# ilirlikalla/Smith-Waterman-FPGA-module

Hardware: AMD Instinct MI355X
Metric: GCUPS (higher is better)
Workload: dtype f16

## Files before the change

smith-waterman-fpga-module_amd/csrc/swbank_f16_rows.inc:

```
#define SWK_F16M_L_Z0_L0 \
  "v_perm_b32 %[S1], %[nv], %[tb0], %[sel]\n\t" \
  "v_pk_add_f16 %[Db], %[h0], %[S1] clamp\n\t" \
  "v_pk_add_f16 %[DN], %[Da], %[no]\n\t" \
  "v_pk_maximum3_f16 %[h0], %[Da], %[up], %[t0]\n\t" \
  "v_pk_maximum3_f16 %[X], %[DN], %[up], %[t0]\n\t" \
  "v_perm_b32 %[S1], %[nv], %[tb1], %[sel]\n\t" \
  "v_pk_add_f16 %[DN], %[Db], %[no]\n\t" \
  "v_pk_add_f16 %[t0], %[X], %[ne]\n\t" \
  "v_pk_add_f16 %[Da], %[h1], %[S1] clamp\n\t" \
  "v_pk_maximum3_f16 %[h1], %[Db], %[t0], %[t1]\n\t" \
  "v_pk_maximum3_f16 %[X], %[DN], %[t0], %[t1]\n\t" \
  "v_pk_maximum3_f16 %[best], %[best], %[h0], %[h1]\n\t" \
  "v_perm_b32 %[S1], %[nv], %[tb2], %[sel]\n\t" \
  "v_pk_add_f16 %[DN], %[Da], %[no]\n\t" \
  "v_pk_add_f16 %[t1], %[X], %[ne]\n\t" \
  "v_pk_add_f16 %[Db], %[h2], %[S1] clamp\n\t" \
  "v_pk_maximum3_f16 %[h2], %[Da], %[t1], %[t2]\n\t" \
  "v_pk_maximum3_f16 %[X], %[DN], %[t1], %[t2]\n\t" \
  "v_perm_b32 %[S1], %[nv], %[tb3], %[sel]\n\t" \
  "v_pk_add_f16 %[DN], %[Db], %[no]\n\t" \
  "v_pk_add_f16 %[t2], %[X], %[ne]\n\t" \
  "v_pk_add_f16 %[Da], %[h3], %[S1] clamp\n\t" \
  "v_pk_maximum3_f16 %[h3], %[Db], %[t2], %[t3]\n\t" \
  "v_pk_maximum3_f16 %[X], %[DN], %[t2], %[t3]\n\t" \
// ... 1417 lines not shown
  "v_pk_add_f16 %[Db], %[h2], %[p2]\n\t" \
  "v_pk_maximum3_f16 %[b0], %[b0], %[m1], %[h1]\n\t" \
  "v_pk_maximum3_f16 %[t2], %[AO], %[t1], %[t2]\n\t" \
  "v_pk_add_f16 %[AO], %[Db], %[no]\n\t" \
  "v_pk_maximum3_f16 %[h2], %[t2], %[Da], %[c2]\n\t" \
  "v_pk_add_f16 %[Da], %[h3], %[p3]\n\t" \
  "v_pk_maximum3_f16 %[b1], %[b1], %[m2], %[h2]\n\t" \
  "v_pk_maximum3_f16 %[t3], %[AO], %[t2], %[t3]\n\t" \
  "v_pk_add_f16 %[b1], %[b1], %[e1]\n\t" \
  "v_pk_add_f16 %[AO], %[Da], %[no]\n\t" \
  "v_pk_maximum3_f16 %[b1], %[b1], %[g3], %[k3]\n\t" \
  "v_pk_maximum3_f16 %[h3], %[t3], %[Db], %[c3]\n\t" \
  "v_pk_add_f16 %[Db], %[h4], %[p4]\n\t" \
  "v_pk_maximum3_f16 %[b1], %[b1], %[m3], %[h3]\n\t" \
  "v_pk_maximum3_f16 %[t4], %[AO], %[t3], %[t4]\n\t" \
  "v_pk_add_f16 %[AO], %[Db], %[no]\n\t" \
  "v_pk_maximum3_f16 %[h4], %[t4], %[Da], %[c4]\n\t" \
  "v_pk_add_f16 %[Da], %[h5], %[p5]\n\t" \
  "v_pk_maximum3_f16 %[b2], %[b2], %[m4], %[h4]\n\t" \
  "v_pk_maximum3_f16 %[t5], %[AO], %[t4], %[t5]\n\t" \
  "v_pk_add_f16 %[b2], %[b2], %[e1]\n\t" \
  "v_pk_add_f16 %[AO], %[Da], %[no]\n\t" \
  "v_pk_maximum3_f16 %[b2], %[b2], %[g5], %[k5]\n\t" \
  "v_pk_maximum3_f16 %[h5], %[t5], %[Db], %[c5]\n\t" \
  "v_pk_add_f16 %[Db], %[h6], %[p6]\n\t" \
  "v_pk_maximum3_f16 %[b2], %[b2], %[m5], %[h5]\n\t" \
  "v_pk_maximum3_f16 %[t6], %[AO], %[t5], %[t6]\n\t" \
  "v_pk_add_f16 %[AO], %[Db], %[no]\n\t" \
  "v_pk_maximum3_f16 %[h6], %[t6], %[Da], %[c6]\n\t" \
  "v_pk_maximum3_f16 %[t7], %[AO], %[t6], %[t7]\n\t" \
  "v_pk_maximum3_f16 %[b3], %[b3], %[m6], %[h6]\n\t" \
  "v_pk_maximum3_f16 %[h7], %[t7], %[Db], %[c7]\n\t" \
  ""
#define SWK_F16M_F_Z0_L0 \
  "v_pk_fma_f16 %[Db], %[fa0], %[fb0], %[h0] op_sel:[0,1,0] op_sel_hi:[1,0,1] clamp\n\t" \
  "v_pk_add_f16 %[DN], %[Da], %[no]\n\t" \
  "v_pk_maximum3_f16 %[h0], %[Da], %[up], %[t0]\n\t" \
  "v_pk_maximum3_f16 %[X], %[DN], %[up], %[t0]\n\t" \
  "v_pk_add_f16 %[DN], %[Db], %[no]\n\t" \
  "v_pk_add_f16 %[t0], %[X], %[ne]\n\t" \
  "v_pk_fma_f16 %[Da], %[fa1], %[fb1], %[h1] op_sel:[0,1,0] op_sel_hi:[1,0,1] clamp\n\t" \
  "v_pk_maximum3_f16 %[h1], %[Db], %[t0], %[t1]\n\t" \
  "v_pk_maximum3_f16 %[X], %[DN], %[t0], %[t1]\n\t" \
  "v_pk_maximum3_f16 %[best], %[best], %[h0], %[h1]\n\t" \
  "v_pk_add_f16 %[DN], %[Da], %[no]\n\t" \
  "v_pk_add_f16 %[t1], %[X], %[ne]\n\t" \
  "v_pk_fma_f16 %[Db], %[fa2], %[fb2], %[h2] op_sel:[0,1,0] op_sel_hi:[1,0,1] clamp\n\t" \
  "v_pk_maximum3_f16 %[h2], %[Da], %[t1], %[t2]\n\t" \
  "v_pk_maximum3_f16 %[X], %[DN], %[t1], %[t2]\n\t" \
  "v_pk_add_f16 %[DN], %[Db], %[no]\n\t" \
  "v_pk_add_f16 %[t2], %[X], %[ne]\n\t" \
  "v_pk_fma_f16 %[Da], %[fa3], %[fb3], %[h3] op_sel:[0,1,0] op_sel_hi:[1,0,1] clamp\n\t" \
  "v_pk_maximum3_f16 %[h3], %[Db], %[t2], %[t3]\n\t" \
  "v_pk_maximum3_f16 %[X], %[DN], %[t2], %[t3]\n\t" \
  "v_pk_maximum3_f16 %[best], %[best], %[h2], %[h3]\n\t" \
  "v_pk_add_f16 %[DN], %[Da], %[no]\n\t" \
  "v_pk_add_f16 %[t3], %[X], %[ne]\n\t" \
  "v_pk_fma_f16 %[Db], %[fa4], %[fb4], %[h4] op_sel:[0,1,0] op_sel_hi:[1,0,1] clamp\n\t" \
  "v_pk_maximum3_f16 %[h4], %[Da], %[t3], %[t4]\n\t" \
  "v_pk_maximum3_f16 %[X], %[DN], %[t3], %[t4]\n\t" \
  "v_pk_add_f16 %[DN], %[Db], %[no]\n\t" \
  "v_pk_add_f16 %[t4], %[X], %[ne]\n\t" \
  "v_pk_fma_f16 %[Da], %[fa5], %[fb5], %[h5] op_sel:[0,1,0] op_sel_hi:[1,0,1] clamp\n\t" \
  "v_pk_maximum3_f16 %[h5], %[Db], %[t4], %[t5]\n\t" \
  "v_pk_maximum3_f16 %[X], %[DN], %[t4], %[t5]\n\t" \
  "v_pk_maximum3_f16 %[best], %[best], %[h4], %[h5]\n\t" \
// ... 372 lines not shown
```

smith-waterman-fpga-module_amd/csrc/swbank_internal.h:

```cpp
#ifndef SWBANK_INTERNAL_H
#define SWBANK_INTERNAL_H

#define SWB_MAX_QUERY 65536u
#define SWB_TILE 128
#define SWB_SEL_PAD 0x0Du
#define SWB_SEL_ZERO 0x0Cu

#define SWB_RECORD 64
#define SWB_RECORD_MAX 232u

#define SWK_PACK_BYTES 0u
#define SWK_PACK_RECORDS 1u
#define SWK_PACK_STREAM 2u
#define SWK_PACK_NIBBLE 3u
#define SWK_PACK_MIXED 4u

typedef struct SwkWaveSplit {
  unsigned pairs, P;
  const unsigned* qtab;
  const unsigned* fb_qtab;
  unsigned words, fb_words, PS, fb_PS;
  void* ring;
  unsigned cols;
  unsigned* prog;
  unsigned* fault;
  unsigned poll_limit, stall;
  unsigned wbal_blocks, wbal_grid, wbal_gen;
  unsigned wbal_waves;
  unsigned* wbal_flag;
  unsigned* wbal_state;
} SwkWaveSplit;

static inline int swk_wbal_admissible(unsigned long long U, unsigned long long B, unsigned W,
                                      unsigned grid) {
  return (W == 4 || W == 8) && grid != 0 && U * B >= 4ull * W * grid;
}

#define SWK_SKEW_ACC 4
#define SWK_BAL_WORDS(R, ACC) (2 * (R) + 1 + (ACC))

#define SWK_FAULT_BAL 1u
#define SWK_FAULT_TAIL 2u
#define SWK_FAULT_WBAL 4u
#define SWK_FAULT_WORDS 4


typedef struct SwkStreamChunk {
  unsigned tile0, res_off_lo, res_off_hi, zero_off256;
} SwkStreamChunk;
#define SWK_STREAM_ABORT 0xFFFFFFFFu

#define SWK_DEAL_MAX 16
typedef struct SwkDeal {
  unsigned D, stride;
  unsigned char* codes[SWK_DEAL_MAX];
  unsigned long long* offs[SWK_DEAL_MAX];
  unsigned* lens[SWK_DEAL_MAX];
  const int* scores[SWK_DEAL_MAX];
  unsigned long long cnt[SWK_DEAL_MAX];
  unsigned nib;
} SwkDeal;

#ifdef __cplusplus
extern "C"
#endif
int swbank_codon_table(const unsigned char* user, unsigned char out[64]);

#ifdef __cplusplus
extern "C" hipError_t swk_launch_stream(int R, int gotoh, int f16, int pair, const uint8_t* res,
                                        size_t n, uint32_t ulen, const SwkStreamChunk* sc,
                                        const uint32_t* hflag, uint32_t* dflag, uint32_t nsc,
// ... 15 lines not shown
```

smith-waterman-fpga-module_amd/csrc/swbank_ktile.hip:

```cpp
#include "swbank_kcommon.h"

namespace swk {

template <int C>
__device__ __forceinline__ void tile_chunks_local(const Lane2& t, size_t tlo, size_t thi, size_t n,
                                                  int lane, int& nch, int& nfull, int& ncl) {
  uint32_t Lmax = max(t.llo, t.lhi);
  uint32_t Lmin = min(tlo < n ? t.llo : ~0u, thi < n ? t.lhi : ~0u);
  uint32_t ol = (uint32_t)lane;
  asm volatile("" : "+v"(ol));
#pragma unroll
  for (int off = 32; off >= 1; off >>= 1) {
    const int ad = (int)((ol ^ (uint32_t)off) << 2);
    Lmax = max(Lmax, (uint32_t)__builtin_amdgcn_ds_bpermute(ad, (int)Lmax));
    Lmin = min(Lmin, (uint32_t)__builtin_amdgcn_ds_bpermute(ad, (int)Lmin));
  }
  const int lx = (int)__builtin_amdgcn_readfirstlane(Lmax);
  nch = max(1, (lx + C - 1) / C);
  ncl = lx == 0 ? C : lx - C * (nch - 1);
  const uint32_t lm = __builtin_amdgcn_readfirstlane(Lmin);
  nfull = lm == ~0u ? 0 : (int)(lm / C);
}

template <int R, int RB, bool COL0, bool PROF, bool GOTOH, bool F16, bool PAIR = false,
          bool MQ = false, bool STREAM = false, int C = 8, bool BAL = false, bool TRIM = false,
          bool SKEW = false>
__global__ void __launch_bounds__(R >= 64 ? 512 : 1024) score_kernel(const ScoreArgs a) {
  static_assert(!BAL || (!MQ && !STREAM && !COL0), "balanced ranges: one query, resident batch");
  static_assert(!TRIM || (BAL && PAIR), "trimmed last chunks: the balanced pair kernel");
  static_assert(!SKEW || (PAIR && F16 && !GOTOH && !MQ && !STREAM && R == 32 && C == 8),
                "SKEW: the merged f16 pair rows, one query, resident batch");
  static_assert(!MQ || !PROF, "several queries: row-LUT or pair-table variants");
  static_assert(!STREAM || (!MQ && !PROF), "streamed batches: single-query LUT / pair variants");
  static_assert(C == 8 || (C == 4 && PAIR && !STREAM), "4-column chunks: pair tables only");
  static_assert(!PAIR || ((R == 32 || (R == 16 && GOTOH)) && F16 && !PROF && !COL0 &&
                          (!GOTOH || !MQ)),
                "PAIR: f16, merged R = 32 or Gotoh R = 16 / 32 (one query)");
  extern __shared__ __attribute__((aligned(16))) uint32_t smem[];
  const int lane = threadIdx.x & 63;
  const int wave = __builtin_amdgcn_readfirstlane(threadIdx.x >> 6);
  const int W = __builtin_amdgcn_readfirstlane(blockDim.x >> 6);
  const bool seg_in = a.edge_in != nullptr, seg_out = a.edge_out != nullptr;
  uint32_t* bestsh = smem + (PAIR ? a.PS / 4 : 0);
  constexpr int RS = SWK_RING_ROW;
  uint2* ein = reinterpret_cast<uint2*>(bestsh + W * SWB_TILE);
  uint2* ring = ein + (seg_in ? 2 * C * RS : 0);
  uint8_t* prof = reinterpret_cast<uint8_t*>(ring + (size_t)(W > 1 ? 2 * (W - 1) : 1) * C * RS);

  size_t n = a.n;
  const uint32_t* idx = a.idx;
  if (idx && a.ident && __builtin_amdgcn_readfirstlane(*a.ident)) idx = nullptr;
  const uint32_t* sidx = TRIM ? a.sidx : nullptr;
  if (TRIM && sidx && a.ident && __builtin_amdgcn_readfirstlane(*a.ident)) sidx = nullptr;
  if (idx) {
    const uint32_t cnt = __builtin_amdgcn_readfirstlane(*a.nidx);
    n = cnt > a.idx_base ? min(a.n, (size_t)(cnt - a.idx_base)) : 0;
  }
  const int ntiles = (int)((n + SWB_TILE - 1) / SWB_TILE);
  const int G = (int)gridDim.x;
// ... 85 lines not shown
      return lane_targets<true>(base + (((size_t)scn * 12 + 15) & ~(size_t)15),
                                reinterpret_cast<const uint64_t*>(co), cl, scn, t - st0, lane, pk,
                                cperm, 0u, 0u);
    }
    return lane_targets<true>(base, nullptr, nullptr, scn, t - st0, lane, pk, nullptr, a.ulen,
                               pk == SWK_PACK_NIBBLE ? (a.ulen + 1) / 2 : (a.ulen + 3) / 4);
  };

  int unit = blockIdx.x, q = 0;
  int tile = unit;
  int vc0 = 0, vend = 0;
  if constexpr (BAL) {
    bal_visit(0, tile, vc0, vend);
    unit = tile;
  }
  if constexpr (MQ) {
    if (unit < nunits) {
      q = PAIR ? unit % (int)a.nq : unit / ntiles;
      tile = PAIR ? unit / (int)a.nq : unit - q * ntiles;
    }
  }
  Lane2 cur;
  if constexpr (STREAM) {
    cur = stream_tile(tile, packed);
    wperm = cperm;
    wst0 = st0;
  } else {
    cur = lane_targets<!MQ>(a.res, a.offs, a.lens, n, tile, lane, packed, idx, a.ulen,
                            a.ustride);
  }
  int nch, nfull, ncl;
  if constexpr (SKEW)
    tile_chunks_local<C>(cur, (size_t)tile * SWB_TILE + lane, (size_t)tile * SWB_TILE + lane + 64,
                         n, lane, nch, nfull, ncl);
  else
    tile_chunks<C>(cur, (size_t)tile * SWB_TILE + lane, (size_t)tile * SWB_TILE + lane + 64, n,
                   nch, nfull, ncl);
  (void)ncl;
  if constexpr (BAL) {
    if (vend >= 0 && vend < nch) ncl = C;
    nch = vend < 0 ? nch : vend;
  }
  const uint32_t S = a.S;

  for (int i = threadIdx.x; i < W * SWB_TILE; i += blockDim.x) bestsh[i] = 0;
  const f16x2 NOE2 = as_f16x2(as_u16x2(a.f16_noe)), NE2 = as_f16x2(as_u16x2(a.f16_ne)),
              NO2 = as_f16x2(as_u16x2(a.f16_no));
  typedef __attribute__((address_space(4))) const uint32_t cst_u32;
  cst_u32* const ct = reinterpret_cast<cst_u32*>(reinterpret_cast<uintptr_t>(a.ctab));
  constexpr uint32_t SKEW_NEG = 0xBC00BC00u;
  constexpr int NB = SKEW ? SWK_SKEW_ACC : 1;
  static_assert(NB == 1 || NB == 4, "the generated rows fold into 4 accumulators");
  uint32_t skew_c0 = 0;
  if constexpr (SKEW) skew_c0 = ct[1];
  const auto skew_reset = [&](u16x2 (&H)[R], u16x2 (&X)[R], u16x2 (&bk)[NB], u16x2& pup) {
    uint32_t c0 = skew_c0;
    asm volatile("" : "+v"(c0));
    f16x2 h = as_f16x2(__builtin_bit_cast(u16x2, c0));
    const f16x2 ne = as_f16x2(as_u16x2(a.f16_ne));
#pragma unroll
    for (int r = 0; r < R; ++r) {
      if (r < 8) {
        H[r] = as_u16x2(h);
        h = h - ne;
      } else {
        H[r] = H[r - 8];
      }
      X[r] = __builtin_bit_cast(u16x2, SKEW_NEG);
    }
    pup = H[7];
    if constexpr (NB == 4) {
      bk[0] = H[1];
      bk[1] = H[3];
      bk[2] = H[5];
      bk[3] = H[6];
    }
  };
  (void)ct; (void)skew_reset;
  if (wave == 0) {
    if (lane < C)
      ring[lane * RS + 64] = F16 ? make_uint2(0u, GOTOH ? 0u : as_u32(as_u16x2(NOE2)))
                                 : make_uint2(S | (S << 16), 0u);
    if (seg_in)
      dma_edge_chunk<C>(a.edge_in + (size_t)(MQ ? unit : tile) * a.ecols * 64, ein, lane);
  }
  uint32_t nv = a.nv;
  uint32_t tab[PROF || PAIR ? 1 : R];
  if constexpr (PAIR) {
    const uint4* src = reinterpret_cast<const uint4*>(a.qtab + (MQ ? (size_t)q * a.qwords : 0));
    for (uint32_t i = threadIdx.x; i < a.PS / 16; i += blockDim.x)
      reinterpret_cast<uint4*>(smem)[i] = src[i];
  } else if constexpr (PROF) {
    const uint32_t words = (a.pad + 1) * a.PS / 16;
    const uint4* src = reinterpret_cast<const uint4*>(a.qtab);
    for (uint32_t i = threadIdx.x; i < words; i += blockDim.x)
      reinterpret_cast<uint4*>(prof)[i] = src[i];
  } else {
    asm volatile("" : "+v"(nv));
#pragma unroll
    for (int r = 0; r < R; ++r)
      tab[r] = __builtin_amdgcn_readfirstlane(a.qtab[(MQ ? (size_t)q * a.qwords : 0) + wave * R + r]);
  }
  const u16x2 S2 = {(unsigned short)S, (unsigned short)S};
  const u16x2 O2 = {(unsigned short)a.O, (unsigned short)a.O};
  const u16x2 E2 = {(unsigned short)a.E, (unsigned short)a.E};
  const uint32_t oes = a.O + a.E + S;
  const u16x2 OES2 = {(unsigned short)oes, (unsigned short)oes};
  const u16x2 H0 = F16 ? (u16x2){0, 0} : S2;
  const u16x2 X0 = (F16 && !GOTOH) ? as_u16x2(NOE2) : (u16x2){0, 0};

  u16x2 Hl[R], Xl[R];
#pragma unroll
  for (int r = 0; r < R; ++r) {
    Hl[r] = H0;
    Xl[r] = X0;
// ... 140 lines not shown
            if (lane == 0) {
              sq[(k + 1) % W] = nt;
              if (nt >= ntiles) sq[W] = g + 1;
            }
            nunit = nt;
          } else {
            nunit = __builtin_amdgcn_readfirstlane(sq[(k + 1) % W]);
          }
        }
      }
      int ntile = nunit, nqq = q;
      if constexpr (MQ) {
        if (nunit < nunits) {
          if constexpr (PAIR) {
            ntile = nunit / (int)a.nq;
          } else {
            ntile = tile + G;
            while (ntile >= ntiles) {
              ntile -= ntiles;
              ++nqq;
            }
          }
        }
      }
      if (!last) {
        load_raw<C, !MQ>(cur, c + 1, c + 1 < nfull, a.pad, packed, rlo, rhi);
      } else if (nunit < nunits) {
        if constexpr (STREAM) cur = stream_tile(ntile, packed_n);
        else
          cur = lane_targets<!MQ>(a.res, a.offs, a.lens, n, ntile, lane, packed, idx, a.ulen,
                                  a.ustride);
        if constexpr (SKEW)
          tile_chunks_local<C>(cur, (size_t)ntile * SWB_TILE + lane,
                               (size_t)ntile * SWB_TILE + lane + 64, n, lane, nch_n, nfull_n, ncl_n);
        else
          tile_chunks<C>(cur, (size_t)ntile * SWB_TILE + lane,
                         (size_t)ntile * SWB_TILE + lane + 64, n, nch_n, nfull_n, ncl_n);
        if (BAL && nvend >= 0 && nvend < nch_n) ncl_n = C;
        if (BAL && nvend < 0) nvend = nch_n;
        load_raw<C, !MQ>(cur, nc0, nc0 < nfull_n, a.pad, STREAM ? packed_n : packed, rlo, rhi);
      }
      const int slot = g & 1;
      if (seg_in && wave == 0 && (last ? nunit < nunits : (MQ ? unit : tile) < nunits))
        dma_edge_chunk<C>(a.edge_in + ((size_t)(last ? nunit : MQ ? unit : tile) * a.ecols +
                                    (size_t)(last ? 0 : c + 1) * C) * 64,
                       ein + (size_t)((g + 1) & 1) * C * RS, lane);
      int rl = lane;
      if constexpr (SKEW) asm volatile("" : "+v"(rl));
      uint2* rin = wave > 0 ? ring + ((size_t)((wave - 1) * 2 + slot) * C) * RS + rl
                   : seg_in ? ein + (size_t)slot * C * RS + rl
                            : ring + 64;
      uint2* rout = wave < W - 1 ? ring + ((size_t)(wave * 2 + slot) * C) * RS + rl
                    : W > 1      ? rin
                                 : ring + rl;
      const int cu = __builtin_amdgcn_readfirstlane(c);
      uint32_t cs[SKEW ? 7 + C : 1];
      if constexpr (SKEW) {
        cst_u32* const sl = ct + (cu * C + 2);
#pragma unroll
        for (int s = 0; s < 7 + C; ++s) cs[s] = sl[s];
        if (wave == 0 && lane == 0) {
#pragma unroll
          for (int jj = 0; jj < C; ++jj) ring[jj * RS + 64] = make_uint2(cs[jj + 7], SKEW_NEG);
        }
      }
      (void)cu; (void)cs;
      uint2 rv = rin[0];
      ProfLookup16<PROF && F16 ? R : 2> lkq;
      (void)lkq;
      const int ncols = TRIM && c + 1 == nch ? ncl : C;
      bool trimmed = false;
      (void)ncols;
#pragma unroll
      for (int jj = 0; jj < C; ++jj) {
        if (TRIM && jj > 0 && __builtin_expect(jj >= ncols, 0)) {
          trimmed = true;
          break;
        }
        const u16x2 upH = as_u16x2(rv.x);
        u16x2 upX = as_u16x2(rv.y);
        if (jj + 1 < C) rv = rin[(jj + 1) * RS];
        u16x2 diag = prevUpH;
        prevUpH = upH;
        const uint32_t wlo = jj < 4 ? clo.x : clo.y, whi = jj < 4 ? chi.x : chi.y;
        if constexpr (PROF && F16) {
          const auto load16 = [&](int j, ProfLookup16<R>& out) {
            const uint32_t wl = j < 4 ? clo.x : clo.y, wh = j < 4 ? chi.x : chi.y;
            const uint32_t blo = min((wl >> (8 * (j & 3))) & 0xFFu, padc);
            const uint32_t bhi = min((wh >> (8 * (j & 3))) & 0xFFu, padc);
            const uint4* plo = reinterpret_cast<const uint4*>(prof + __umul24(blo, a.PS) + 2 * pbase);
            const uint4* phi = reinterpret_cast<const uint4*>(prof + __umul24(bhi, a.PS) + 2 * pbase);
#pragma unroll
            for (int q = 0; q < R / 8; ++q) {
              const uint4 x = plo[q], y = phi[q];
              out.lo[4 * q] = x.x; out.lo[4 * q + 1] = x.y; out.lo[4 * q + 2] = x.z;
              out.lo[4 * q + 3] = x.w;
// ... 9 lines not shown
          if (COL0 && jj == 0 && c == 0)
            column_f16<R, RB, GOTOH, true>(lk, diag, upX, Hl, Xl, best, NOE2, NE2, NO2);
          else
            column_f16<R, RB, GOTOH, false>(lk, diag, upX, Hl, Xl, best, NOE2, NE2, NO2);
        } else if constexpr (PROF) {
          ProfLookup<R> lk;
          const uint32_t blo = min((wlo >> (8 * (jj & 3))) & 0xFFu, padc);
          const uint32_t bhi = min((whi >> (8 * (jj & 3))) & 0xFFu, padc);
          const uint4* plo = reinterpret_cast<const uint4*>(prof + __umul24(blo, a.PS) + pbase);
          const uint4* phi = reinterpret_cast<const uint4*>(prof + __umul24(bhi, a.PS) + pbase);
#pragma unroll
          for (int q = 0; q < R / 16; ++q) {
            const uint4 x = plo[q], y = phi[q];
            lk.lo[4 * q] = x.x; lk.lo[4 * q + 1] = x.y; lk.lo[4 * q + 2] = x.z;
            lk.lo[4 * q + 3] = x.w;
            lk.hi[4 * q] = y.x; lk.hi[4 * q + 1] = y.y; lk.hi[4 * q + 2] = y.z;
            lk.hi[4 * q + 3] = y.w;
          }
          __builtin_amdgcn_sched_barrier(0);
          if constexpr (GOTOH) {
            u16x2 uH = upH;
            column_gotoh<R, RB>(lk, diag, uH, upX, Hl, Xl, best, S2, OES2, E2);
          } else if (COL0 && jj == 0 && c == 0) {
            column_merged<R, RB, true>(lk, diag, upX, Hl, Xl, best, S2, O2, E2);
          } else {
            column_merged<R, RB, false>(lk, diag, upX, Hl, Xl, best, S2, O2, E2);
          }
        } else if constexpr (PAIR && SKEW) {
          const uint32_t nwl = jj + 1 < C ? (jj + 1 < 4 ? clo.x : clo.y) : rlo.x;
          const uint32_t nwh = jj + 1 < C ? (jj + 1 < 4 ? chi.x : chi.y) : rhi.x;
          const int nsh = jj + 1 < C ? 8 * ((jj + 1) & 3) : 0;
          uint32_t Da, Db, AO;
          const uint32_t no = as_u32(as_u16x2(NO2)), e1 = a.f16_e1, ne8 = a.f16_ne8;
#define SWK_SKEW_OUT(B, DA, DB)                                                               \
  [h0] "+v"(Hl[B]), [h1] "+v"(Hl[B + 1]), [h2] "+v"(Hl[B + 2]), [h3] "+v"(Hl[B + 3]),          \
      [h4] "+v"(Hl[B + 4]), [h5] "+v"(Hl[B + 5]), [h6] "+v"(Hl[B + 6]), [h7] "+v"(Hl[B + 7]),  \
      [t0] "+v"(Xl[B]), [t1] "+v"(Xl[B + 1]), [t2] "+v"(Xl[B + 2]), [t3] "+v"(Xl[B + 3]),      \
      [t4] "+v"(Xl[B + 4]), [t5] "+v"(Xl[B + 5]), [t6] "+v"(Xl[B + 6]), [t7] "+v"(Xl[B + 7]),  \
      [Db] DB(Db), [Da] DA(Da), [AO] DA(AO)
#define SWK_SKEW_IN(P0, P1)                                                                   \
  [p0] "v"(P0.x), [p1] "v"(P0.y), [p2] "v"(P0.z), [p3] "v"(P0.w), [p4] "v"(P1.x),             \
      [p5] "v"(P1.y), [p6] "v"(P1.z), [p7] "v"(P1.w), [no] "s"(no), [ne8] "s"(ne8),           \
      [c0] "s"(cs[jj]), [c1] "s"(cs[jj + 1]), [c2] "s"(cs[jj + 2]), [c3] "s"(cs[jj + 3]),     \
      [c4] "s"(cs[jj + 4]), [c5] "s"(cs[jj + 5]), [c6] "s"(cs[jj + 6]), [c7] "s"(cs[jj + 7])
#define SWK_SKEW_FOLD(N, B)                                                                   \
  [N##0] "v"(Hl[B]), [N##1] "v"(Hl[B + 1]), [N##2] "v"(Hl[B + 2]), [N##3] "v"(Hl[B + 3]),     \
      [N##4] "v"(Hl[B + 4]), [N##5] "v"(Hl[B + 5]), [N##6] "v"(Hl[B + 6])
          uint4 pB0 = ld4(acur + 48), pB1 = ld4(acur + 64);
          __builtin_amdgcn_sched_barrier(0);
          asm volatile(SWK_F16SKEW_F
                       : SWK_SKEW_OUT(0, "=&v", "=&v"), [up] "+v"(upX), [b3] "+v"(bk[3])
                       : SWK_SKEW_IN(pA0, pA1), [e1] "s"(e1), [dg] "v"(diag), [pw] "v"(pw),
                         [x] "v"(Hl[15]), [y] "v"(Hl[23]), [z] "v"(Hl[31]));
          pA0 = ld4(acur + 80);
          pA1 = ld4(acur + 96);
          __builtin_amdgcn_sched_barrier(0);
          asm volatile(SWK_F16SKEW_M : SWK_SKEW_OUT(8, "+v", "+v") : SWK_SKEW_IN(pB0, pB1));
          pB0 = ld4(acur + 112);
          pB1 = ld4(acur + 128);
          __builtin_amdgcn_sched_barrier(0);
          asm volatile(SWK_F16SKEW_M : SWK_SKEW_OUT(16, "+v", "+v") : SWK_SKEW_IN(pA0, pA1));
          acur = pair_addr(nwl, nwh, nsh);
          pA0 = ld4(acur + 16);
          pA1 = ld4(acur + 32);
          pw = ld1(acur + 12);
          __builtin_amdgcn_sched_barrier(0);
          asm volatile(SWK_F16SKEW_L
                       : SWK_SKEW_OUT(R - 8, "+v", "+v"), [b0] "+v"(bk[0]), [b1] "+v"(bk[1]),
                         [b2] "+v"(bk[2]), [b3] "+v"(bk[3])
                       : SWK_SKEW_IN(pB0, pB1), [e1] "s"(e1), SWK_SKEW_FOLD(g, 0),
                         SWK_SKEW_FOLD(k, 8), SWK_SKEW_FOLD(m, 16));
#undef SWK_SKEW_FOLD
#undef SWK_SKEW_OUT
#undef SWK_SKEW_IN
          (void)Db; (void)AO; (void)Da;
          upX = Xl[R - 1];
        } else if constexpr (PAIR) {
          const uint32_t nwl = jj + 1 < C ? (jj + 1 < 4 ? clo.x : clo.y) : rlo.x;
          const uint32_t nwh = jj + 1 < C ? (jj + 1 < 4 ? chi.x : chi.y) : rhi.x;
          const int nsh = jj + 1 < C ? 8 * ((jj + 1) & 3) : 0;
          uint32_t Da, Db, X, DN, IN;
          const uint32_t noe = as_u32(as_u16x2(NOE2)), ne = as_u32(as_u16x2(NE2)),
                 no = as_u32(as_u16x2(NO2));
          u16x2 bst = best;
          u16x2 F = upX;
#define SWK_PAIR_HT(B)                                                                        \
  [h0] "+v"(Hl[B]), [h1] "+v"(Hl[B + 1]), [h2] "+v"(Hl[B + 2]), [h3] "+v"(Hl[B + 3]),          \
      [h4] "+v"(Hl[B + 4]), [h5] "+v"(Hl[B + 5]), [h6] "+v"(Hl[B + 6]), [h7] "+v"(Hl[B + 7]),  \
      [t0] "+v"(Xl[B]), [t1] "+v"(Xl[B + 1]), [t2] "+v"(Xl[B + 2]), [t3] "+v"(Xl[B + 3]),      \
      [t4] "+v"(Xl[B + 4]), [t5] "+v"(Xl[B + 5]), [t6] "+v"(Xl[B + 6]), [t7] "+v"(Xl[B + 7]),  \
      [Db] "=&v"(Db), [best] "+v"(bst)
#define SWK_PAIR_OUT(B, DA) SWK_PAIR_HT(B), [Da] DA(Da), [X] "=&v"(X), [DN] "=&v"(DN), [IN] "=&v"(IN)
#define SWK_PAIR_OUTG(B, DA)                                                                  \
  SWK_PAIR_HT(B), [Da] DA(Da), [EN] "=&v"(X), [HN] "=&v"(DN), [FN] "=&v"(IN), [F] "+v"(F)
#define SWK_PAIR_IN(P0, P1)                                                                   \
  [p0] "v"(P0.x), [p1] "v"(P0.y), [p2] "v"(P0.z), [p3] "v"(P0.w), [p4] "v"(P1.x),             \
      [p5] "v"(P1.y), [p6] "v"(P1.z), [p7] "v"(P1.w), [noe] "s"(noe), [ne] "s"(ne), [no] "s"(no)
#define SWK_PAIR_BLOCK(KIND, B, P0, P1)                                                       \
  if constexpr (GOTOH) {                                                                      \
    if constexpr (KIND == 0)                                                                  \
      asm volatile(SWK_F16PAIRG_F : SWK_PAIR_OUTG(B, "=&v")                                   \
                   : SWK_PAIR_IN(P0, P1), [dg] "v"(diag), [pw] "v"(pw));                   \
    else if constexpr (KIND == 1)                                                             \
      asm volatile(SWK_F16PAIRG_M : SWK_PAIR_OUTG(B, "+v") : SWK_PAIR_IN(P0, P1));         \
// ... 51 lines not shown
          __builtin_amdgcn_sched_barrier(0);
          if constexpr (GOTOH) {
            u16x2 uH = upH;
            column_gotoh<R, RB>(lk, diag, uH, upX, Hl, Xl, best, S2, OES2, E2);
          } else if (COL0 && jj == 0 && c == 0) {
            column_merged<R, RB, true>(lk, diag, upX, Hl, Xl, best, S2, O2, E2);
          } else {
            column_merged<R, RB, false>(lk, diag, upX, Hl, Xl, best, S2, O2, E2);
          }
        }
        if constexpr (!SKEW) asm volatile("" : "+v"(best));
        rout[jj * RS] = make_uint2(as_u32(Hl[R - 1]), as_u32(upX));
      }
      if constexpr (PAIR && TRIM) {
        if (trimmed) {
          acur = pair_addr(rlo.x, rhi.x, 0);
          pA0 = ld4(acur + 16);
          pA1 = ld4(acur + 32);
          pw = ld1(acur + 12);
        }
      }
      (void)trimmed;
      if (seg_out && wave == W - 1) {
        uint2* dst = a.edge_out + ((size_t)(MQ ? unit : tile) * a.ecols + (size_t)c * C) * 64 + lane;
#pragma unroll
        for (int jj = 0; jj < C; ++jj) dst[jj * 64] = rout[jj * RS];
      }
      if (last) {
        if (BAL && k == 0 && bf > 0) {
          bal_store((int)blockIdx.x + 1);
        } else {
        if constexpr (SKEW) {
          const f16x2 e1 = as_f16x2(as_u16x2(a.f16_e1));
          f16x2 bb = fmax2(fmax2(as_f16x2(bk[3]) + e1, as_f16x2(Hl[7])), as_f16x2(Hl[15]));
          bb = fmax2(fmax2(bb, as_f16x2(Hl[23])), as_f16x2(Hl[31]));
          f16x2 lo = fmax2((as_f16x2(bk[0]) + e1) + e1, as_f16x2(bk[1]));
          lo = fmax2((lo + e1) + e1, as_f16x2(bk[2]));
          bb = fmax2((lo + e1) + e1, bb);
          const uint32_t cf = ct[__builtin_amdgcn_readfirstlane(cu * C + ncols + 8)];
          best = as_u16x2(bb - as_f16x2(__builtin_bit_cast(u16x2, cf)));
        }
        uint32_t* bs = bestsh + (k % W) * SWB_TILE;
        if constexpr (SKEW) {
          uint32_t ol = (uint32_t)lane;
          asm volatile("" : "+v"(ol));
          bs += ol;
        } else {
          bs += lane;
        }
        atomicMax(&bs[0], (uint32_t)best.x);
        atomicMax(&bs[64], (uint32_t)best.y);
        if (wave == W - 1) {
          const size_t tlo = (size_t)tile * SWB_TILE + lane, thi = tlo + 64;
          int32_t blo = (int32_t)bs[0], bhi = (int32_t)bs[64];
          bs[0] = 0;
          bs[64] = 0;
          if constexpr (F16) {
            blo = f16_unscore((uint32_t)blo);
            bhi = f16_unscore((uint32_t)bhi);
          }
          const uint32_t* sx = TRIM && sidx ? sidx : idx;
          size_t slo = sx && tlo < n ? sx[tlo] : tlo;
          size_t shi = sx && thi < n ? sx[thi] : thi;
          if constexpr (STREAM) {
            if (wperm) {
              const size_t b0 = (size_t)wst0 * SWB_TILE;
              if (tlo < n) slo = b0 + wperm[tlo - b0];
              if (thi < n) shi = b0 + wperm[thi - b0];
            }
          }
          int32_t* qsc = MQ ? a.scores + (size_t)q * a.sstride : a.scores;
// ... 353 lines not shown
```

smith-waterman-fpga-module_amd/csrc/swbank_launch.hip:

```cpp
#include "swbank_bank.h"

static bool one_len_bin(uint32_t min_len, uint32_t max_len) {
  if (min_len > max_len) return false;
  uint32_t shift = 0;
  while ((max_len >> shift) >= 2048u) ++shift;
  return ((max_len - min_len) >> shift) == 0;
}

void u16_gotoh_rows(const sw_bank* b, bool f16, int& R, int& W) {
  if (f16 || !b->gotoh() || b->prof || R != 32 || b->segs.size() != 1 || b->query.size() > 256)
    return;
  R = 16;
  W = std::max(1, (int)((b->query.size() + 15) / 16));
}

bool wave_preferred(const sw_bank* b, size_t n, uint32_t max_len, bool use_f16) {
  const size_t nseg = b->segs.size();
  const size_t ntiles = (n + SWB_TILE - 1) / SWB_TILE;
  const bool gotoh = b->cfg.gap_model == SW_GAP_GOTOH;
  const double tiles = (double)ntiles, W = b->segs[0].W;
  const double cu_frac = std::min(1.0, tiles / 256.0);
  const double wps = std::min(4.0, std::max(1.0, std::ceil(tiles / 256.0)) * W / 4.0);
  const bool pair_tab = use_f16 && b->pair_bytes != 0 && env_int("SWBANK_PAIR", 1) != 0;
  const double tile_base = use_f16 ? (gotoh ? (b->prof ? 7100 : pair_tab ? 8500 : 7500)
// ... 304 lines not shown
            if (b->bal_key[0] != ntiles || b->bal_key[1] != K || b->bal_key[2] != grid) {
              HIPOK(b, b->bal_plan.reserve((size_t)(grid + 1) * 4));
              HIPOK(b, swk_bal_plan_uniform(b->bal_plan.p, (uint32_t)ntiles, (uint32_t)K, grid,
                                            st));
              b->bal_key[0] = ntiles;
              b->bal_key[1] = K;
              b->bal_key[2] = grid;
            }
          }
          const int gmode = rbal && ragged_trim() && packed == SWK_PACK_BYTES
                                ? env_int("SWBANK_RAGGED_GATHER", 0) : 0;
          const bool gat = gmode != 0;
          const bool gnib = gat && gmode == 2 && b->alpha <= 16;
          SwkDeal dl{};
          if (gat) {
            const size_t stride = ((gnib ? ((size_t)max_len + 7) / 8 * 4 : (size_t)max_len) + 15) &
                                  ~(size_t)15;
            HIPOK(b, b->gres.reserve(n * stride + 16));
            HIPOK(b, b->goffs.reserve(n));
            HIPOK(b, b->glens.reserve(n));
            dl.D = 1;
            dl.stride = (unsigned)stride;
            dl.codes[0] = b->gres.p;
            dl.offs[0] = reinterpret_cast<unsigned long long*>(b->goffs.p);
            dl.lens[0] = b->glens.p;
            dl.cnt[0] = n;
            dl.nib = gnib ? 1u : 0u;
            HIPOK(b, swk_deal_gather(res, offs, lens, idx, ident, n, &dl, st));
          }
          HIPOK(b, swk_launch_pair_bal(gat ? b->gres.p : res, gat ? b->goffs.p : offs,
                                       gat ? b->glens.p : lens, np,
                                       skew ? b->qpair_skew.p : b->qpair.p, b->nv16, b->S, b->O,
                                       b->E, b->pair_bytes, b->pad, Wl,
                                       scores, b->pS1, b->pS2, ulen,
                                       ustride, b->bal_flag.p, b->bal_state.p, ++b->bal_gen, grid,
                                       gat ? nullptr : idx, gat ? nullptr : nidx,
                                       ident, b->bal_plan.p,
                                       fw + (b->host_call ? SWK_FAULT_WORDS : 0), poll_limit(1u << 23),
                                       (uint32_t)std::max(0, env_int("SWBANK_STALL", 0)),
                                       rbal && ragged_trim(),
                                       gnib ? (uint32_t)SWK_PACK_NIBBLE
                                            : gat ? (uint32_t)SWK_PACK_BYTES : packed,
                                       gat ? idx : nullptr, st,
                                       skew ? b->skew_ctab.p : nullptr));
          ++b->ctr.balanced_calls;
          const size_t L = strlen(b->last_kernel);
          snprintf(b->last_kernel + L, sizeof(b->last_kernel) - L, " balanced grid=%u%s", grid,
                   gnib ? " gather4" : gat ? " gather" : "");
          continue;
        }
      }
      for (size_t s = 0; s < nseg; ++s) {
        const void* ein = s > 0 ? b->edge[(s - 1) & 1].p : nullptr;
        void* eout = s + 1 < nseg ? b->edge[s & 1].p : nullptr;
        const bool pair = f16 && use_pair;
        int R = b->R, Wl = b->segs[s].W;
        u16_gotoh_rows(b, f16, R, Wl);
        HIPOK(b, swk_launch_score(R, b->RB, b->col0, b->prof, gotoh ? 1 : 0, f16 ? 1 : 0, res,
                                  offs, lens, np,
                                  pair && skew ? b->qpair_skew.p
                                  : pair       ? b->qpair.p + s * (b->pair_bytes / 4)
                                  : f16 ? b->qtab16.p + b->segs[s].off16
                                        : b->qtab.p + b->segs[s].off,
                                  f16 ? b->nv16 : b->nv, b->S, b->O, b->E,
                                  pair ? b->pair_bytes : f16 && b->prof ? b->PS16 : b->PS,
                                  b->pad, Wl, scores, ein, eout, ecols, s > 0 ? 1 : 0,
                                  (int)packed, idx, nidx, (uint32_t)p0,
// ... 234 lines not shown
```

Baseline: 14510.

## Use eight rotating skew accumulators and skip wave reduction for uniform lengths

For non-trimmed skew kernels, the running-best accumulators grow from 4 to 8 and are renamed by column index within a chunk. The per-chunk fold then needs fewer dependent add/max steps, and some gap-extension bookkeeping moves into the asm. When a uniform length is known, the chunk-count computation skips the cross-lane bpermute max/min reduction. The launcher now passes max_len as ulen in some cases. The extra accumulators raise register pressure, and the ring-slot initialization and store semantics change (atomic store of only .x).

```diff
diff --git a/smith-waterman-fpga-module_amd/csrc/swbank_f16_rows.inc b/smith-waterman-fpga-module_amd/csrc/swbank_f16_rows.inc
--- a/smith-waterman-fpga-module_amd/csrc/swbank_f16_rows.inc
+++ b/smith-waterman-fpga-module_amd/csrc/swbank_f16_rows.inc
@@ -1473,6 +1473,93 @@
   "v_pk_maximum3_f16 %[b3], %[b3], %[m6], %[h6]\n\t" \
   "v_pk_maximum3_f16 %[h7], %[t7], %[Db], %[c7]\n\t" \
   ""
+#define SWK_F16SKEW8_F \
+  "v_pk_add_f16 %[Da], %[dg], %[pw]\n\t" \
+  "v_pk_add_f16 %[up], %[up], %[ne8]\n\t" \
+  "v_pk_add_f16 %[Db], %[h0], %[p0]\n\t" \
+  "v_pk_add_f16 %[AO], %[Da], %[no]\n\t" \
+  "v_pk_add_f16 %[bm], %[bm], %[ne8] neg_lo:[0,1] neg_hi:[0,1]\n\t" \
+  "v_pk_maximum3_f16 %[t0], %[AO], %[up], %[t0]\n\t" \
+  "v_pk_add_f16 %[AO], %[Db], %[no]\n\t" \
+  "v_pk_maximum3_f16 %[bf], %[bf], %[h7], %[x]\n\t" \
+  "v_pk_maximum3_f16 %[h0], %[t0], %[Da], %[c0]\n\t" \
+  "v_pk_add_f16 %[Da], %[h1], %[p1]\n\t" \
+  "v_pk_maximum3_f16 %[t1], %[AO], %[t0], %[t1]\n\t" \
+  "v_pk_maximum3_f16 %[bf], %[bf], %[y], %[z]\n\t" \
+  "v_pk_add_f16 %[AO], %[Da], %[no]\n\t" \
+  "v_pk_maximum3_f16 %[h1], %[t1], %[Db], %[c1]\n\t" \
+  "v_pk_add_f16 %[Db], %[h2], %[p2]\n\t" \
+  "v_pk_maximum3_f16 %[t2], %[AO], %[t1], %[t2]\n\t" \
+  "v_pk_add_f16 %[AO], %[Db], %[no]\n\t" \
+  "v_pk_maximum3_f16 %[h2], %[t2], %[Da], %[c2]\n\t" \
+  "v_pk_add_f16 %[Da], %[h3], %[p3]\n\t" \
+  "v_pk_maximum3_f16 %[t3], %[AO], %[t2], %[t3]\n\t" \
+  "v_pk_add_f16 %[AO], %[Da], %[no]\n\t" \
+  "v_pk_maximum3_f16 %[h3], %[t3], %[Db], %[c3]\n\t" \
+  "v_pk_add_f16 %[Db], %[h4], %[p4]\n\t" \
+  "v_pk_maximum3_f16 %[t4], %[AO], %[t3], %[t4]\n\t" \
+  "v_pk_add_f16 %[AO], %[Db], %[no]\n\t" \
+  "v_pk_maximum3_f16 %[h4], %[t4], %[Da], %[c4]\n\t" \
+  "v_pk_add_f16 %[Da], %[h5], %[p5]\n\t" \
+  "v_pk_maximum3_f16 %[t5], %[AO], %[t4], %[t5]\n\t" \
+  "v_pk_add_f16 %[AO], %[Da], %[no]\n\t" \
+  "v_pk_maximum3_f16 %[h5], %[t5], %[Db], %[c5]\n\t" \
+  "v_pk_add_f16 %[Db], %[h6], %[p6]\n\t" \
+  "v_pk_maximum3_f16 %[t6], %[AO], %[t5], %[t6]\n\t" \
+  "v_pk_add_f16 %[AO], %[Db], %[no]\n\t" \
+  "v_pk_maximum3_f16 %[h6], %[t6], %[Da], %[c6]\n\t" \
+  "v_pk_add_f16 %[Da], %[h7], %[p7]\n\t" \
+  "v_pk_maximum3_f16 %[t7], %[AO], %[t6], %[t7]\n\t" \
+  "v_pk_add_f16 %[AO], %[Da], %[no]\n\t" \
+  "v_pk_maximum3_f16 %[h7], %[t7], %[Db], %[c7]\n\t" \
+  "v_pk_add_f16 %[Db], %[t7], %[ne8]\n\t" \
+  ""
+#define SWK_F16SKEW8_L \
+  "v_pk_maximum3_f16 %[t0], %[AO], %[Db], %[t0]\n\t" \
+  "v_pk_maximum3_f16 %[b0], %[b0], %[g0], %[k0]\n\t" \
+  "v_pk_add_f16 %[Db], %[h0], %[p0]\n\t" \
+  "v_pk_maximum3_f16 %[b1], %[b1], %[g1], %[k1]\n\t" \
+  "v_pk_maximum3_f16 %[h0], %[t0], %[Da], %[c0]\n\t" \
+  "v_pk_maximum3_f16 %[b2], %[b2], %[g2], %[k2]\n\t" \
+  "v_pk_add_f16 %[AO], %[Db], %[no]\n\t" \
+  "v_pk_maximum3_f16 %[b3], %[b3], %[g3], %[k3]\n\t" \
+  "v_pk_add_f16 %[Da], %[h1], %[p1]\n\t" \
+  "v_pk_maximum3_f16 %[b4], %[b4], %[g4], %[k4]\n\t" \
+  "v_pk_maximum3_f16 %[t1], %[AO], %[t0], %[t1]\n\t" \
+  "v_pk_maximum3_f16 %[b5], %[b5], %[g5], %[k5]\n\t" \
+  "v_pk_add_f16 %[AO], %[Da], %[no]\n\t" \
+  "v_pk_maximum3_f16 %[b6], %[b6], %[g6], %[k6]\n\t" \
+  "v_pk_maximum3_f16 %[h1], %[t1], %[Db], %[c1]\n\t" \
+  "v_pk_maximum3_f16 %[b0], %[b0], %[m0], %[h0]\n\t" \
+  "v_pk_add_f16 %[Db], %[h2], %[p2]\n\t" \
+  "v_pk_maximum3_f16 %[b1], %[b1], %[m1], %[h1]\n\t" \
+  "v_pk_maximum3_f16 %[t2], %[AO], %[t1], %[t2]\n\t" \
+  "v_pk_add_f16 %[AO], %[Db], %[no]\n\t" \
+  "v_pk_maximum3_f16 %[h2], %[t2], %[Da], %[c2]\n\t" \
+  "v_pk_add_f16 %[Da], %[h3], %[p3]\n\t" \
+  "v_pk_maximum3_f16 %[b2], %[b2], %[m2], %[h2]\n\t" \
+  "v_pk_maximum3_f16 %[t3], %[AO], %[t2], %[t3]\n\t" \
+  "v_pk_add_f16 %[AO], %[Da], %[no]\n\t" \
+  "v_pk_maximum3_f16 %[h3], %[t3], %[Db], %[c3]\n\t" \
+  "v_pk_add_f16 %[Db], %[h4], %[p4]\n\t" \
+  "v_pk_maximum3_f16 %[b3], %[b3], %[m3], %[h3]\n\t" \
+  "v_pk_maximum3_f16 %[t4], %[AO], %[t3], %[t4]\n\t" \
+  "v_pk_add_f16 %[AO], %[Db], %[no]\n\t" \
+  "v_pk_maximum3_f16 %[h4], %[t4], %[Da], %[c4]\n\t" \
+  "v_pk_add_f16 %[Da], %[h5], %[p5]\n\t" \
+  "v_pk_maximum3_f16 %[b4], %[b4], %[m4], %[h4]\n\t" \
+  "v_pk_maximum3_f16 %[t5], %[AO], %[t4], %[t5]\n\t" \
+  "v_pk_add_f16 %[AO], %[Da], %[no]\n\t" \
+  "v_pk_maximum3_f16 %[h5], %[t5], %[Db], %[c5]\n\t" \
+  "v_pk_add_f16 %[Db], %[h6], %[p6]\n\t" \
+  "v_pk_maximum3_f16 %[b5], %[b5], %[m5], %[h5]\n\t" \
+  "v_pk_maximum3_f16 %[t6], %[AO], %[t5], %[t6]\n\t" \
+  "v_pk_add_f16 %[AO], %[Db], %[no]\n\t" \
+  "v_pk_maximum3_f16 %[h6], %[t6], %[Da], %[c6]\n\t" \
+  "v_pk_maximum3_f16 %[t7], %[AO], %[t6], %[t7]\n\t" \
+  "v_pk_maximum3_f16 %[b6], %[b6], %[m6], %[h6]\n\t" \
+  "v_pk_maximum3_f16 %[h7], %[t7], %[Db], %[c7]\n\t" \
+  ""
 #define SWK_F16M_F_Z0_L0 \
   "v_pk_fma_f16 %[Db], %[fa0], %[fb0], %[h0] op_sel:[0,1,0] op_sel_hi:[1,0,1] clamp\n\t" \
   "v_pk_add_f16 %[DN], %[Da], %[no]\n\t" \
diff --git a/smith-waterman-fpga-module_amd/csrc/swbank_internal.h b/smith-waterman-fpga-module_amd/csrc/swbank_internal.h
--- a/smith-waterman-fpga-module_amd/csrc/swbank_internal.h
+++ b/smith-waterman-fpga-module_amd/csrc/swbank_internal.h
@@ -36,7 +36,8 @@
   return (W == 4 || W == 8) && grid != 0 && U * B >= 4ull * W * grid;
 }
 
-#define SWK_SKEW_ACC 4
+#define SWK_SKEW_ACC 8
+#define SWK_SKEW_ACC_TRIM 4
 #define SWK_BAL_WORDS(R, ACC) (2 * (R) + 1 + (ACC))
 
 #define SWK_FAULT_BAL 1u
diff --git a/smith-waterman-fpga-module_amd/csrc/swbank_ktile.hip b/smith-waterman-fpga-module_amd/csrc/swbank_ktile.hip
--- a/smith-waterman-fpga-module_amd/csrc/swbank_ktile.hip
+++ b/smith-waterman-fpga-module_amd/csrc/swbank_ktile.hip
@@ -4,7 +4,16 @@
 
 template <int C>
 __device__ __forceinline__ void tile_chunks_local(const Lane2& t, size_t tlo, size_t thi, size_t n,
-                                                  int lane, int& nch, int& nfull, int& ncl) {
+                                                  int lane, int& nch, int& nfull, int& ncl,
+                                                  int tile, uint32_t ulen) {
+  if (ulen) {
+    const bool any = (size_t)tile * SWB_TILE < n;
+    const int lx = any ? (int)ulen : 0;
+    nch = max(1, (lx + C - 1) / C);
+    ncl = lx == 0 ? C : lx - C * (nch - 1);
+    nfull = lx / C;
+    return;
+  }
   uint32_t Lmax = max(t.llo, t.lhi);
   uint32_t Lmin = min(tlo < n ? t.llo : ~0u, thi < n ? t.lhi : ~0u);
   uint32_t ol = (uint32_t)lane;
@@ -24,7 +33,7 @@
 
 template <int R, int RB, bool COL0, bool PROF, bool GOTOH, bool F16, bool PAIR = false,
           bool MQ = false, bool STREAM = false, int C = 8, bool BAL = false, bool TRIM = false,
-          bool SKEW = false>
+          bool SKEW = false, int NB = SKEW ? (TRIM ? SWK_SKEW_ACC_TRIM : SWK_SKEW_ACC) : 1>
 __global__ void __launch_bounds__(R >= 64 ? 512 : 1024) score_kernel(const ScoreArgs a) {
   static_assert(!BAL || (!MQ && !STREAM && !COL0), "balanced ranges: one query, resident batch");
   static_assert(!TRIM || (BAL && PAIR), "trimmed last chunks: the balanced pair kernel");
@@ -176,7 +185,7 @@
   int nch, nfull, ncl;
   if constexpr (SKEW)
     tile_chunks_local<C>(cur, (size_t)tile * SWB_TILE + lane, (size_t)tile * SWB_TILE + lane + 64,
-                         n, lane, nch, nfull, ncl);
+                         n, lane, nch, nfull, ncl, tile, TRIM ? 0u : a.ulen);
   else
     tile_chunks<C>(cur, (size_t)tile * SWB_TILE + lane, (size_t)tile * SWB_TILE + lane + 64, n,
                    nch, nfull, ncl);
@@ -193,8 +202,8 @@
   typedef __attribute__((address_space(4))) const uint32_t cst_u32;
   cst_u32* const ct = reinterpret_cast<cst_u32*>(reinterpret_cast<uintptr_t>(a.ctab));
   constexpr uint32_t SKEW_NEG = 0xBC00BC00u;
-  constexpr int NB = SKEW ? SWK_SKEW_ACC : 1;
-  static_assert(NB == 1 || NB == 4, "the generated rows fold into 4 accumulators");
+  static_assert(SKEW ? (NB == 4 || (NB == 8 && !TRIM)) : NB == 1,
+                "the generated rows fold into 4 accumulators, or 8 renamed over a whole chunk");
   uint32_t skew_c0 = 0;
   if constexpr (SKEW) skew_c0 = ct[1];
   const auto skew_reset = [&](u16x2 (&H)[R], u16x2 (&X)[R], u16x2 (&bk)[NB], u16x2& pup) {
@@ -218,13 +227,18 @@
       bk[1] = H[3];
       bk[2] = H[5];
       bk[3] = H[6];
+    } else if constexpr (NB == 8) {
+#pragma unroll
+      for (int i = 0; i < 7; ++i) bk[i] = H[i + 1];
+      bk[7] = H[0];
     }
   };
   (void)ct; (void)skew_reset;
   if (wave == 0) {
     if (lane < C)
-      ring[lane * RS + 64] = F16 ? make_uint2(0u, GOTOH ? 0u : as_u32(as_u16x2(NOE2)))
-                                 : make_uint2(S | (S << 16), 0u);
+      ring[lane * RS + 64] = SKEW && !TRIM ? make_uint2(0u, SKEW_NEG)
+                             : F16 ? make_uint2(0u, GOTOH ? 0u : as_u32(as_u16x2(NOE2)))
+                                   : make_uint2(S | (S << 16), 0u);
     if (seg_in)
       dma_edge_chunk<C>(a.edge_in + (size_t)(MQ ? unit : tile) * a.ecols * 64, ein, lane);
   }
@@ -431,7 +445,8 @@
                                   a.ustride);
         if constexpr (SKEW)
           tile_chunks_local<C>(cur, (size_t)ntile * SWB_TILE + lane,
-                               (size_t)ntile * SWB_TILE + lane + 64, n, lane, nch_n, nfull_n, ncl_n);
+                               (size_t)ntile * SWB_TILE + lane + 64, n, lane, nch_n, nfull_n, ncl_n,
+                               ntile, TRIM ? 0u : a.ulen);
         else
           tile_chunks<C>(cur, (size_t)ntile * SWB_TILE + lane,
                          (size_t)ntile * SWB_TILE + lane + 64, n, nch_n, nfull_n, ncl_n);
@@ -460,7 +475,14 @@
         for (int s = 0; s < 7 + C; ++s) cs[s] = sl[s];
         if (wave == 0 && lane == 0) {
 #pragma unroll
-          for (int jj = 0; jj < C; ++jj) ring[jj * RS + 64] = make_uint2(cs[jj + 7], SKEW_NEG);
+          for (int jj = 0; jj < C; ++jj) {
+            if constexpr (TRIM)
+              ring[jj * RS + 64] = make_uint2(cs[jj + 7], SKEW_NEG);
+            else
+              __atomic_store_n(reinterpret_cast<__attribute__((address_space(3))) uint32_t*>(
+                                   (size_t)(lds_void_ptr)&ring[jj * RS + 64].x),
+                               cs[jj + 7], __ATOMIC_RELAXED);
+          }
         }
       }
       (void)cu; (void)cs;
@@ -536,6 +558,7 @@
           const int nsh = jj + 1 < C ? 8 * ((jj + 1) & 3) : 0;
           uint32_t Da, Db, AO;
           const uint32_t no = as_u32(as_u16x2(NO2)), e1 = a.f16_e1, ne8 = a.f16_ne8;
+          (void)e1;
 #define SWK_SKEW_OUT(B, DA, DB)                                                               \
   [h0] "+v"(Hl[B]), [h1] "+v"(Hl[B + 1]), [h2] "+v"(Hl[B + 2]), [h3] "+v"(Hl[B + 3]),          \
       [h4] "+v"(Hl[B + 4]), [h5] "+v"(Hl[B + 5]), [h6] "+v"(Hl[B + 6]), [h7] "+v"(Hl[B + 7]),  \
@@ -552,10 +575,17 @@
       [N##4] "v"(Hl[B + 4]), [N##5] "v"(Hl[B + 5]), [N##6] "v"(Hl[B + 6])
           uint4 pB0 = ld4(acur + 48), pB1 = ld4(acur + 64);
           __builtin_amdgcn_sched_barrier(0);
-          asm volatile(SWK_F16SKEW_F
-                       : SWK_SKEW_OUT(0, "=&v", "=&v"), [up] "+v"(upX), [b3] "+v"(bk[3])
-                       : SWK_SKEW_IN(pA0, pA1), [e1] "s"(e1), [dg] "v"(diag), [pw] "v"(pw),
-                         [x] "v"(Hl[15]), [y] "v"(Hl[23]), [z] "v"(Hl[31]));
+          if constexpr (NB == 8)
+            asm volatile(SWK_F16SKEW8_F
+                         : SWK_SKEW_OUT(0, "=&v", "=&v"), [up] "+v"(upX),
+                           [bf] "+v"(bk[(jj + 6) & 7]), [bm] "+v"(bk[(jj + 7) & 7])
+                         : SWK_SKEW_IN(pA0, pA1), [dg] "v"(diag), [pw] "v"(pw),
+                           [x] "v"(Hl[15]), [y] "v"(Hl[23]), [z] "v"(Hl[31]));
+          else
+            asm volatile(SWK_F16SKEW_F
+                         : SWK_SKEW_OUT(0, "=&v", "=&v"), [up] "+v"(upX), [b3] "+v"(bk[3 % NB])
+                         : SWK_SKEW_IN(pA0, pA1), [e1] "s"(e1), [dg] "v"(diag), [pw] "v"(pw),
+                           [x] "v"(Hl[15]), [y] "v"(Hl[23]), [z] "v"(Hl[31]));
           pA0 = ld4(acur + 80);
           pA1 = ld4(acur + 96);
           __builtin_amdgcn_sched_barrier(0);
@@ -569,11 +599,20 @@
           pA1 = ld4(acur + 32);
           pw = ld1(acur + 12);
           __builtin_amdgcn_sched_barrier(0);
-          asm volatile(SWK_F16SKEW_L
-                       : SWK_SKEW_OUT(R - 8, "+v", "+v"), [b0] "+v"(bk[0]), [b1] "+v"(bk[1]),
-                         [b2] "+v"(bk[2]), [b3] "+v"(bk[3])
-                       : SWK_SKEW_IN(pB0, pB1), [e1] "s"(e1), SWK_SKEW_FOLD(g, 0),
-                         SWK_SKEW_FOLD(k, 8), SWK_SKEW_FOLD(m, 16));
+          if constexpr (NB == 8)
+            asm volatile(SWK_F16SKEW8_L
+                         : SWK_SKEW_OUT(R - 8, "+v", "+v"), [b0] "+v"(bk[jj & 7]),
+                           [b1] "+v"(bk[(jj + 1) & 7]), [b2] "+v"(bk[(jj + 2) & 7]),
+                           [b3] "+v"(bk[(jj + 3) & 7]), [b4] "+v"(bk[(jj + 4) & 7]),
+                           [b5] "+v"(bk[(jj + 5) & 7]), [b6] "+v"(bk[(jj + 6) & 7])
+                         : SWK_SKEW_IN(pB0, pB1), SWK_SKEW_FOLD(g, 0), SWK_SKEW_FOLD(k, 8),
+                           SWK_SKEW_FOLD(m, 16));
+          else
+            asm volatile(SWK_F16SKEW_L
+                         : SWK_SKEW_OUT(R - 8, "+v", "+v"), [b0] "+v"(bk[0]), [b1] "+v"(bk[1 % NB]),
+                           [b2] "+v"(bk[2 % NB]), [b3] "+v"(bk[3 % NB])
+                         : SWK_SKEW_IN(pB0, pB1), [e1] "s"(e1), SWK_SKEW_FOLD(g, 0),
+                           SWK_SKEW_FOLD(k, 8), SWK_SKEW_FOLD(m, 16));
 #undef SWK_SKEW_FOLD
 #undef SWK_SKEW_OUT
 #undef SWK_SKEW_IN
@@ -691,11 +730,21 @@
         } else {
         if constexpr (SKEW) {
           const f16x2 e1 = as_f16x2(as_u16x2(a.f16_e1));
-          f16x2 bb = fmax2(fmax2(as_f16x2(bk[3]) + e1, as_f16x2(Hl[7])), as_f16x2(Hl[15]));
-          bb = fmax2(fmax2(bb, as_f16x2(Hl[23])), as_f16x2(Hl[31]));
-          f16x2 lo = fmax2((as_f16x2(bk[0]) + e1) + e1, as_f16x2(bk[1]));
-          lo = fmax2((lo + e1) + e1, as_f16x2(bk[2]));
-          bb = fmax2((lo + e1) + e1, bb);
+          f16x2 bb;
+          if constexpr (NB == 8) {
+            bb = as_f16x2(bk[7]);
+#pragma unroll
+            for (int i = 0; i < 6; ++i) bb = fmax2(bb + e1, as_f16x2(bk[i]));
+            f16x2 b6 = fmax2(fmax2(as_f16x2(bk[6]), as_f16x2(Hl[7])), as_f16x2(Hl[15]));
+            b6 = fmax2(fmax2(b6, as_f16x2(Hl[23])), as_f16x2(Hl[31]));
+            bb = fmax2(bb + e1, b6);
+          } else {
+            bb = fmax2(fmax2(as_f16x2(bk[3 % NB]) + e1, as_f16x2(Hl[7])), as_f16x2(Hl[15]));
+            bb = fmax2(fmax2(bb, as_f16x2(Hl[23])), as_f16x2(Hl[31]));
+            f16x2 lo = fmax2((as_f16x2(bk[0]) + e1) + e1, as_f16x2(bk[1 % NB]));
+            lo = fmax2((lo + e1) + e1, as_f16x2(bk[2 % NB]));
+            bb = fmax2((lo + e1) + e1, bb);
+          }
           const uint32_t cf = ct[__builtin_amdgcn_readfirstlane(cu * C + ncols + 8)];
           best = as_u16x2(bb - as_f16x2(__builtin_bit_cast(u16x2, cf)));
         }
diff --git a/smith-waterman-fpga-module_amd/csrc/swbank_launch.hip b/smith-waterman-fpga-module_amd/csrc/swbank_launch.hip
--- a/smith-waterman-fpga-module_amd/csrc/swbank_launch.hip
+++ b/smith-waterman-fpga-module_amd/csrc/swbank_launch.hip
@@ -360,7 +360,8 @@
                                        gat ? b->glens.p : lens, np,
                                        skew ? b->qpair_skew.p : b->qpair.p, b->nv16, b->S, b->O,
                                        b->E, b->pair_bytes, b->pad, Wl,
-                                       scores, b->pS1, b->pS2, ulen,
+                                       scores, b->pS1, b->pS2,
+                                       ustride || rbal ? ulen : max_len,
                                        ustride, b->bal_flag.p, b->bal_state.p, ++b->bal_gen, grid,
                                        gat ? nullptr : idx, gat ? nullptr : nidx,
                                        ident, b->bal_plan.p,
```

Result: faster. 14810, median of 6 (+2.1%).
